# CZW123456/Quantized_Decoder_Polar_Codes

Measured on AMD Instinct MI355X. Metric: decoded frames/sec (N=1024, SCL-LUT L=8, Q=16) at 1/2/4/8 GPUs; BER match, higher is better.
Workload: dtype u8; 1 GPU; SCL-LUT N=1024 K=512 L=8 Q=16 (5G-NR PW code, no CRC); decoder=SCL-LUT, N=1024, K=512, L=8, v=16, luts=mindistortion, parallelism=dp1 (frames sharded by global frame id, RCCL counter all-reduce), engine=fast, lds_bytes_per_wave=7424, lds_from_depth=5, ops=266, prefix_ops=65, waves=5120

## Files before the change

### quantized_decoder_polar_codes_amd/csrc/qpd_capi_build.hpp

```cpp
#pragma once
#include <cstdlib>
#include <cstring>
#include <map>

#include "qpd_config.hpp"
#include "qpd_decoder.hpp"
#include "qpd_plan.hpp"
#include "qpd_schedule.hpp"

namespace qpd {
const void *fast_kernel_single(int kind, int sets);
const void *prefix_kernel(int kind, int sets, bool pw1);
const void *fast_kernel_scl(int sets, bool l8, bool w16);
const void *fast_kernel_scl_pw1(int sets, bool l8, bool w16);
const void *fast_kernel_fscl(int sets, bool l8, bool r1l);
const void *fast_kernel_fscl_pw1(int sets, bool l8, bool r1l);
const void *fast_kernel_fscl_w16(int sets, bool pw1);
const void *generic_kernel(int fam, int dom, bool wide);
const void *generic_list_kernel(int fam, int dom, bool wide);
const void *dmetric_kernel();
const void *fast_kernel_scl_st(int sets, bool l8, bool w16);
const void *fast_kernel_scl_pw1_st(int sets, bool l8, bool w16);
const void *fast_kernel_fscl_st(int sets, bool l8, bool r1l);
const void *fast_kernel_fscl_pw1_st(int sets, bool l8, bool r1l);
const void *fast_kernel_fscl_w16_st(int sets, bool pw1);
const void *fast_kernel_scl_ls(int sets, bool l8, bool w16);
const void *fast_kernel_scl_pw1_ls(int sets, bool l8, bool w16);
// ... 27 lines not shown
            default: return nullptr;
        }
    }
    switch (kind) {
        case QPD_SC_LUT:
        case QPD_FASTSC_LUT: return pw1 || r1l ? nullptr : qpd::fast_kernel_single(kind, sets);
        case QPD_SCL_LUT: return r1l ? nullptr : pw1 ? qpd::fast_kernel_scl_pw1(sets, l8, w16) : qpd::fast_kernel_scl(sets, l8, w16);
        case QPD_FASTSCL_LUT:
            if (w16) return r1l ? nullptr : qpd::fast_kernel_fscl_w16(sets, pw1);
            return pw1 ? qpd::fast_kernel_fscl_pw1(sets, l8, r1l) : qpd::fast_kernel_fscl(sets, l8, r1l);
        default: return nullptr;
    }
}
using qpd::generic_kernel;
using qpd::prefix_kernel;

int init_task_queue(qpd_decoder *d) {
    uint32_t v0 = 0;
    if (const char *e = getenv("QPD_TASK_BASE0")) v0 = (uint32_t)strtoull(e, nullptr, 0);
    const uint32_t init[2] = {v0, 0u};
    const int rc = upload(d->task_ctr, init, 2, d->hs);
    if (rc) return rc;
    d->task_base = v0;
    return QPD_OK;
}

#ifdef QPD_STAMPS
unsigned long long *stamp_buffer() {
    static std::mutex mu;
    static std::map<int, unsigned long long *> bufs;
// ... 138 lines not shown
    d->lds_bytes = H.lds_bytes;
    d->lds_tab_bytes = H.lds_tab_bytes;
    d->sets = H.sets;
    d->pfx_sets = H.pfx_sets;
    d->l8 = H.l8;
    d->w16 = H.w16;
    d->r1l = H.r1l;
    d->pw1 = H.pw1;
    d->pre = H.pre;
    d->pre_chunk = H.pre_chunk;
    for (int i = 0; i < 3; ++i) {
        d->pfx[i].nops = (int)H.pfx[i].size();
        d->pfx[i].rec = H.pfx_rec[i], d->pfx[i].pm = H.pfx_pm[i];
        d->pfx[i].paths = 1 << i;
    }
    F.nops = (int)H.ops.size();
    d->num_mops = F.nops + d->prefix_ops();
}

int upload_fast_plan(qpd_decoder *d, const qpd_plan::FastHostPlan &H) {
    int rc;
    if ((rc = upload(d->r1_rank, H.r1tab.data(), H.r1tab.size(), d->hs))) return rc;
    for (const auto &st : H.pfx)
        d->pfx_ops_host.insert(d->pfx_ops_host.end(), st.begin(), st.end());
    if (!d->pfx_ops_host.empty()) {
        if ((rc = upload(d->pfx_mops, d->pfx_ops_host.data(), d->pfx_ops_host.size(), d->hs))) return rc;
        d->main_ops_host = H.ops;
    }
    if ((rc = upload(d->mops, H.ops.data(), H.ops.size(), d->hs))) return rc;
    if ((rc = upload(d->f_tab, H.ft.data(), H.ft.size(), d->hs))) return rc;
    return upload(d->g_tab, H.gt.data(), H.gt.size(), d->hs);
}

int build_fast(qpd_decoder *d, const qpd_config *c, const Schedule &s) {
    qpd::FastPlan &F = d->fplan;
#ifdef QPD_STAMPS
    F.stamps = stamp_buffer();
#endif
    qpd_plan::FastHostPlan H;
    std::string err;
    int rc = qpd_plan::plan_fast(*c, d->n, d->L, s, qpd_plan::PlanSwitches::from_env(), H, err);
    if (rc) return fail(rc, err);
    adopt_fast_plan(d, c, s, H);
    if ((rc = upload_fast_plan(d, H))) return rc;
    const void *kfn = fast_kernel(d->kind, d->sets, d->l8, d->r1l, d->pw1, d->w16);
    if (!kfn) return fail(QPD_E_UNSUPPORTED, "fast plan: no decode kernel instantiation for this plan");
    if ((rc = check_no_static_lds(kfn, "fast decode kernel"))) return rc;
    if (d->kind == QPD_SCL_LUT || d->kind == QPD_FASTSCL_LUT) {
        const void *ksfn = fast_kernel(d->kind, d->sets, d->l8, d->r1l, d->pw1, d->w16, 1);
        if (!ksfn) return fail(QPD_E_UNSUPPORTED, "fast plan: no decode-status kernel instantiation for this plan");
        if ((rc = check_no_static_lds(ksfn, "fast decode-status kernel"))) return rc;
        if (d->L > 1 && d->L <= qpd_list::kMaxListOut) {
            const void *klfn = fast_kernel(d->kind, d->sets, d->l8, d->r1l, d->pw1, d->w16, 2);
            if (!klfn) return fail(QPD_E_UNSUPPORTED, "fast plan: no list-output kernel instantiation for this plan");
            if ((rc = check_no_static_lds(klfn, "fast list-output kernel"))) return rc;
        }
    }
    if (d->pfx[0].nops > 0 && d->pfx_sets == 2 &&
        (rc = check_no_static_lds(prefix_kernel(d->kind, d->pfx_sets, d->pw1), "fast prefix kernel")))
        return rc;
    const int64_t per_wave = (int64_t)d->sets * F.glb_rows * 64 * 4;
    int mw = c->max_waves;
    if (mw <= 0) {
        int per_cu = 0;
        const int ncu = device_cus();
        const hipError_t oe = hipOccupancyMaxActiveBlocksPerMultiprocessor(&per_cu, kfn, 64, d->lds_bytes);
        if (oe != hipSuccess || per_cu <= 0) per_cu = 16;
        mw = std::max(1, ncu) * per_cu;
    }
    mw = (int)std::max<int64_t>(1, std::min<int64_t>(mw, ((int64_t)2 << 30) / per_wave));
    d->max_waves = mw;
    d->scratch_bytes_per_wave = per_wave;
    QPD_HIP(hipMalloc(&d->fscratch.p, (size_t)per_wave * mw));
    F.r1_rank = (const uint16_t *)d->r1_rank.p;
    F.f_tab = (const uint32_t *)d->f_tab.p;
    F.g_tab = (const uint32_t *)d->g_tab.p;
// ... 88 lines not shown
```

### quantized_decoder_polar_codes_amd/csrc/qpd_capi_decode.hpp

```cpp
#pragma once
#include "qpd_capi_build.hpp"
#include "qpd_decoder.hpp"
#include "qpd_fast_pre.hpp"

namespace {

int import_stage(const qpd::MOp &m) { return m.node == 3 ? 1 : m.node == 2 ? 2 : 0; }

int patch_imports(qpd_decoder *d, hipStream_t st) {
    bool moved = false;
    for (const auto &sg : d->pfx) moved = moved || sg.patched != sg.buf.p;
    if (!moved) return QPD_OK;
    auto patch = [&](std::vector<qpd::MOp> &v) {
        for (qpd::MOp &m : v)
            if (m.type == qpd::OP_IMPORT && (m.flags & qpd::MF_XBUF)) {
                const uint64_t a = (uint64_t)(uintptr_t)d->pfx[import_stage(m)].buf.p;
                m.u_row = (int32_t)(uint32_t)a;
                m.r_row = (int32_t)(uint32_t)(a >> 32);
            }
    };
    patch(d->pfx_ops_host);
    patch(d->main_ops_host);
    QPD_HIP(hipMemcpyAsync(d->pfx_mops.p, d->pfx_ops_host.data(), d->pfx_ops_host.size() * sizeof(qpd::MOp),
                           hipMemcpyHostToDevice, st));
// ... 52 lines not shown
    qpd::DevPlan P = d->plan;
    P.task_base = d->task_base;
    status_at(d, out, P);
    list_at(d, out, P);
    const In *in_arg = in;
    void *args[] = {&P, &in_arg, &B, &out, &dmetric};
    const int rc = timed_launch(d, QPD_KC_DECODE, st, [&]() -> int {
        QPD_HIP(hipLaunchKernel(kfn, dim3(grid), dim3(64), args, 0, st));
        QPD_HIP(hipGetLastError());
        return QPD_OK;
    });
    if (!rc) d->task_base += (uint32_t)((B + d->plan.fpw - 1) / d->plan.fpw);
    return rc;
}

int fast_launch(qpd_decoder *d, qpd::FastPlan fp, const int32_t *in, int64_t Bc, uint8_t *out, hipStream_t st,
                bool prefix = false) {
    const int sets = prefix ? d->pfx_sets : d->sets;
    const int64_t tw = (int64_t)fp.fpw * sets;
    const bool status = !prefix && d->st_req.any(), list = !prefix && d->ls_req.any();
    const void *kfn = prefix ? prefix_kernel(d->kind, sets, d->pw1)
                             : fast_kernel(d->kind, d->sets, d->l8, d->r1l, d->pw1, d->w16, list ? 2 : status ? 1 : 0);
    if (!kfn) return fail(QPD_E_INVALID, "bad kind");
    qpd::FastStatus so{};
    if (status) status_at(d, out, so);
    if (list) list_at(d, out, so);
    const int64_t fgroups = (Bc + tw - 1) / tw;
    int fgrid = (int)std::min<int64_t>(fgroups, d->max_waves);
    if (!QPD_DYN) {
        const int64_t rounds = (fgroups + fgrid - 1) / fgrid;
        fgrid = (int)((fgroups + rounds - 1) / rounds);
    }
    const qpd::MOp *ops_arg = fp.ops;
    fp.task_base = d->task_base;
    void *args[] = {&fp, &in, &Bc, &out, &ops_arg, &so};
    const size_t lds = (size_t)((d->lds_bytes - d->lds_tab_bytes) / d->sets * sets + d->lds_tab_bytes);
    const int rc = timed_launch(d, prefix ? QPD_KC_PFX : QPD_KC_DECODE, st, [&]() -> int {
        QPD_HIP(hipLaunchKernel(kfn, dim3(fgrid), dim3(64), args, lds, st));
        QPD_HIP(hipGetLastError());
        return QPD_OK;
    });
    if (!rc) d->task_base += (uint32_t)fgroups;
    return rc;
}

constexpr int prefix_geo(int ps) { return (6 - ps) | (ps << 8); }
static_assert(prefix_geo(0) == 6 && prefix_geo(1) == (5 | (1 << 8)) && prefix_geo(2) == (4 | (2 << 8)), "stages 1, 1b, 2");

int decode_pre_rows(qpd_decoder *d, const uint32_t *rows, int64_t Bc, uint8_t *out, hipStream_t st) {
    qpd::FastPlan fp = d->fplan;
    fp.in_vec = 1;
    fp.in_shift = fp.n - 2;
    if (d->pfx[0].nops > 0) {
        int rc = QPD_OK;
        for (auto &sg : d->pfx)
            if (!rc && sg.nops > 0) rc = ensure_records(sg.buf, sg.cap, Bc, sg.rec, sg.paths);
        if (!rc) rc = patch_imports(d, st);
        if (rc) return rc;
        qpd::FastPlan pp = fp;
        const qpd::MOp *ops = (const qpd::MOp *)d->pfx_mops.p;
        for (const auto &sg : d->pfx) {
            if (sg.nops > 0) {
                const int ps = __builtin_ctz(sg.paths);
                pp.ops = ops;
                pp.nops = sg.nops;
                pp.gs = pp.L = sg.paths;
                pp.fpw = 64 >> ps;
                pp.pfx = (uint32_t *)sg.buf.p;
                pp.pfx_rec = sg.rec;
                pp.pfx_geo = prefix_geo(ps);
                pp.pm_off = sg.pm;
                if ((rc = fast_launch(d, pp, (const int32_t *)rows, Bc, nullptr, st, true))) return rc;
            }
            ops += sg.nops;
        }
    }
    return fast_launch(d, fp, (const int32_t *)rows, Bc, out, st);
}

int64_t reserve_pre_rows(qpd_decoder *d, int64_t B, int *rc) {
    return d->pre_rows.reserve(std::min<int64_t>(B, d->pre_chunk), (size_t)d->N, "pre-pass rows hipMalloc: ", rc);
}

int64_t reserve_symbols(qpd_decoder *d, DeviceChunk &buf, int64_t B, int64_t lim, const char *what, int *rc) {
    if (!lim) lim = std::max<int64_t>(1, ((int64_t)1 << 30) / ((int64_t)d->N * 4));
    return buf.reserve(std::min<int64_t>(B, lim), (size_t)d->N * sizeof(int32_t), what, rc);
}
// ... 123 lines not shown
```

### quantized_decoder_polar_codes_amd/csrc/qpd_decoder.hpp

```cpp
#pragma once
#include <hip/hip_runtime.h>

#include <algorithm>
#include <cstdint>
#include <memory>
#include <mutex>
#include <string>
#include <utility>
#include <vector>

#include "qpd.h"
#include "qpd_generic.hip"
#include "qpd_fast_plan.hpp"
#include "qpd_chunk.hpp"
#include "qpd_host.hpp"
#include "qpd_status.hpp"
#include "qpd_list.hpp"

namespace {

thread_local std::string g_err;

int fail(int code, const std::string &msg) {
    g_err = msg;
// ... 78 lines not shown
    DevPlan plan{};
    qpd::FastPlan fplan{};
    DeviceBuf f_tab, g_tab, fscratch, mops, r1_rank, task_ctr;
    int num_mops = 0;
    DeviceBuf pfx_mops;
    int pfx_sets = 1;
    struct PrefixStage {
        int nops = 0;
        int rec = 0, pm = 0;
        int paths = 1;
        DeviceBuf buf;
        size_t cap = 0;
        const void *patched = nullptr;
    } pfx[3];
    int prefix_ops() const { return pfx[0].nops + pfx[1].nops + pfx[2].nops; }
    std::vector<qpd::MOp> pfx_ops_host, main_ops_host;
    std::vector<Op> ops_host;
    DeviceBuf lut_f, f_base, lut_g, g_base, vcl, ops, info_pos, scratch, err;
    DeviceBuf r_f, r_g, q_bnd, q_rec, bnd_off, bnd_len, rec_off, rec_len;
    DeviceBuf h_in, h_out, h_st;
    size_t h_in_bytes = 0, h_out_bytes = 0, h_st_bytes = 0;
    hipStream_t hs = nullptr;
    void *pin = nullptr;
    size_t pin_bytes = 0;
    std::mutex mu;
    hipEvent_t last_ev = nullptr;
    hipStream_t last_st = nullptr;
    bool last_valid = false;
    uint32_t task_base = 0;
    std::unique_ptr<qpd_host::Plan> hplan;
// ... 100 lines not shown
```

### quantized_decoder_polar_codes_amd/csrc/qpd_fast.hip

```cpp
#pragma once
#include "qpd_fast_switches.hpp"

#include "qpd_fast_plan.hpp"
#include "qpd_fast_lookup.hpp"
#include "qpd_fast_select.hpp"
#include "qpd_fast_bot.hpp"
#include "qpd_fast_special.hpp"

#define QPD_TAIL_PLAIN 0
#define QPD_TAIL_ST 1
#define QPD_TAIL_LIST 2

#if defined(QPD_LIST_UNIT)
#define QPD_ST QPD_TAIL_LIST
#define QPD_UNIT_FN(f) f##_ls
#elif defined(QPD_STATUS_UNIT)
#define QPD_ST QPD_TAIL_ST
#define QPD_UNIT_FN(f) f##_st
#else
#define QPD_ST QPD_TAIL_PLAIN
#define QPD_UNIT_FN(f) f
#endif

namespace qpd {

template <int KIND, int NS, bool L8, bool R1L = false, bool PFX = false, bool PW1 = false, bool W16 = false,
          int ST = QPD_TAIL_PLAIN>
__global__ __launch_bounds__(64, NS == 3 ? QPD_WPE3
                                : W16 ? QPD_WPE_W16
                                : NS == 2 ? (KIND == K_SCL_LUT && !PFX ? QPD_WPE2_SCL : KIND == K_FASTSCL_LUT ? QPD_WPE2_FSCL : QPD_WPE2)
                                : KIND == K_FASTSCL_LUT ? QPD_WPE_FSCL : QPD_WPE1) void lut_fast_kernel(FastPlan P, const int32_t *__restrict__ in, int64_t B,
                                                               uint8_t *__restrict__ out,
                                                               const MOp *__restrict__ ops, FastStatus SO) {
    constexpr bool kList = (KIND == K_SCL_LUT || KIND == K_FASTSCL_LUT);
    static_assert(!W16 || (!L8 && (KIND == K_SCL_LUT || (KIND == K_FASTSCL_LUT && !R1L && !PFX))),
                  "W16: SCL-LUT / FastSCL-LUT list sizes 9..16");
    static_assert(!ST || (kList && !PFX), "ST: the list kinds' decode kernels");
    constexpr int LM = L8 ? 8 : W16 ? 16 : 0;
    constexpr bool kLazy = QPD_BOT3_LAZY && kList;
    constexpr bool kFast = (KIND == K_FASTSC_LUT || KIND == K_FASTSCL_LUT) && !(QPD_EXP_FSCL & 256);
    constexpr bool kChan = !(PW1 && KIND == K_SCL_LUT);
    extern __shared__ __attribute__((aligned(16))) uint32_t lds_dyn[];
    constexpr bool kLdsTab = kList && NS >= 2 && !QPD_EXP_NO_LDSTAB;
    constexpr int kTabWords = kLdsTab ? 192 : 0;
    uint8_t *const tb = (uint8_t *)lds_dyn;
    uint32_t *const lds_rows = lds_dyn + kTabWords;
    const int sstride = 64;
    int *const sel_all = (int *)(lds_rows + NS * P.lds_rows * 64);
    Mem Mv[NS];
    {
        uint32_t *const slab = P.scratch + (size_t)blockIdx.x * NS * P.glb_rows * 64;
        const __amdgpu_buffer_rsrc_t rs =
            __builtin_amdgcn_make_buffer_rsrc(slab, 0, NS * P.glb_rows * 256 * QPD_EXP_SLABMUL, 0x00020000);
#pragma unroll
        for (int s = 0; s < NS; ++s) {
            Mv[s].lds = lds_rows + s * 64;
            Mv[s].gp = slab + s * 64;
            Mv[s].rs = rs;
            Mv[s].so = s * 256;
            Mv[s].ns = NS;
        }
    }
    const int gs = P.gs;
    const int L = kList ? P.L : 1;
    const int N = P.N;
    const int64_t fpw = P.fpw;
    const int64_t ntasks = (B + NS * fpw - 1) / (NS * fpw);
    const double kInf = __builtin_huge_val();

    for (int64_t task = blockIdx.x; task < ntasks;
         task = QPD_DYN ? (int64_t)gridDim.x + wave_take(P.task_ctr, P.task_base) : task + gridDim.x) {
#ifdef QPD_POISON
        for (int i = threadIdx.x; i < NS * (P.lds_rows * 64 + kSelInts); i += 64) lds_rows[i] = (uint32_t)QPD_POISON;
        for (int r = 0; r < NS * P.glb_rows; ++r) Mv[0].gp[r * 64 + threadIdx.x] = (uint32_t)QPD_POISON;
        wave_sync();
#endif
        PathT<PW1> stv[NS];
        {
            const int lane = threadIdx.x, gl = lane & (gs - 1);
            uint64_t self = 0;
            for (int d = 0; d < kMaxDepth; ++d) self |= (uint64_t)gl << (4 * d);
#pragma unroll
            for (int s = 0; s < NS; ++s) {
                stv[s].pm = (gl == 0) ? 0.0 : kInf;
                stv[s].ps = self;
                stv[s].U() = self;
            }
        }
#ifdef QPD_STAMPS
        uint64_t stamp_acc = 0, stamp_cnt = 0;
#endif
        MOp nxt = ops[0];
        Pre pre = fetch_pre(P, nxt, threadIdx.x, threadIdx.x < P.v ? threadIdx.x : 0);
        for (int oi = 0; oi < P.nops; ++oi) {
            int lane = threadIdx.x;
            asm volatile("" : "+v"(lane));
            const int gl = lane & (gs - 1);
            const int gbase = lane & ~(gs - 1);
            const int vlane = lane < P.v ? lane : 0;
            const int32_t *yv[NS];
            const int gsh = __builtin_ctz(gs);
            if (nxt.flags & (MF_CHAN | MF_PRE)) {
#pragma unroll
                for (int s = 0; s < NS; ++s) {
                    int64_t f = (task * NS + s) * fpw + (lane >> gsh);
                    if (f >= B) f = B - 1;
                    yv[s] = in + (f << P.in_shift);
                }
            } else {
#pragma unroll
                for (int s = 0; s < NS; ++s) yv[s] = in;
            }
            if (nxt.flags & MF_SYNC) wave_sync();
            const MOp op = nxt;
            const Pre cur = pre;
#ifdef QPD_STAMPS
            __builtin_amdgcn_s_waitcnt(0);
            const uint64_t stamp_t0 = __builtin_amdgcn_s_memtime();
#endif
            if (oi + 1 < P.nops) {
                nxt = ops[oi + 1];
                if (!kLazy || op.type != OP_BOT3) pre = fetch_pre(P, nxt, lane, vlane);
            }
            const int fl = op.flags;
            auto run_special = [&]() {
              if constexpr (kFast) {
                  if constexpr (KIND == K_FASTSCL_LUT && L8) {
                    if ((op.type == OP_R0 || op.type == OP_REP) && !(QPD_EXP_FSCL & 512)) {
                        r0rep_multi<kLdsTab, R1L>(P, Mv, op, stv, sel_all, sstride, gl, gbase, lane, cur.T2, tb);
                        return;
                    }
                    if (op.type == OP_R1 && (op.cnt <= stl::kThreshold || (fl & MF_R1_LDS)) && !(QPD_EXP_FSCL & 1024)) {
                        r1_multi<kLdsTab, R1L>(P, Mv, op, stv, sel_all, sstride, gl, gbase, lane, lds_rows, cur.T2, tb);
                        return;
                    }
                    if constexpr (!R1L) return;
// ... 5 lines not shown
                                               L, lane, lds_rows);
                    rotate_sets(stv);
                  }
#else
#pragma unroll
                  for (int s = 0; s < NS; ++s)
                    special_op<kList, LM, R1L>(P, Mv[s], op, stv[s], sel_all + sstride * s, NS * sstride, gl, gbase, L, lane,
                                               lds_rows);
#endif
              }
            };
            switch (op.type) {
                case OP_BOT3:
                    if constexpr (KIND == K_FASTSCL_LUT && L8 && !QPD_EXP_NO_BOTX) {
                        if (fl & MF_BOTX) {
                            if (kLazy && oi + 1 < P.nops) pre = fetch_pre(P, nxt, lane, vlane);
                            botx_op<kLdsTab, kChan>(P, Mv, op, yv, stv, cur.T, cur.T2, gl, gbase, L, sel_all, sstride, lane, tb);
                            break;
                        }
                    }
                    bot3_op<kList, LM, kLazy, kLdsTab, kChan>(P, Mv, op, yv, stv, cur.T, cur.T2, gl, gbase, L, sel_all, sstride, lane, [&]() {
                        if (oi + 1 < P.nops) pre = fetch_pre(P, nxt, lane, vlane);
                    }, tb);
                    break;
                case OP_F:
                case OP_G: {
                    int src[NS], usrc[NS];
#pragma unroll
                    for (int s = 0; s < NS; ++s) {
                        src[s] = gbase + pfield(stv[s].ps, op.sh_src);
                        usrc[s] = gbase + pfield(stv[s].U(), op.sh_u);
                    }
                    if constexpr (kLdsTab) {
                        if (fl & MF_FF) {
                            const int key = ((fl & MF_DST_LDS) ? 1 : 0) | ((fl & MF_FF_DL) ? 2 : 0);
                            stage_tab(tb, cur.T, op.type == OP_F ? (lane & 31) : gtab_dw(lane));
                            stage_tab(tb + 512, cur.T2, lane & 31);
// ... 112 lines not shown
#pragma unroll
                        for (int s = 0; s < NS; ++s) stv[s].U() = pset(stv[s].U(), op.sh_dst, gl);
                    }
                    break;
                }
                case OP_IMPORT:
                    if constexpr (KIND == K_SCL_LUT) {
                        const int live = op.tab2;
#pragma unroll
                        for (int s = 0; s < NS; ++s) {
                            const bool dl = fl & MF_DST_LDS;
                            if (fl & MF_ZERO) {
                                for (int w = 0; w < op.cnt; ++w) Mv[s].st(dl, op.dst_row + w, lane, 0u);
                                continue;
                            }
                            int64_t f = (task * NS + s) * fpw + (lane >> gsh);
                            if (f >= B) f = B - 1;
                            const int G = op.vrow & 255;
                            const uint32_t *src = (const uint32_t *)(((uint64_t)(uint32_t)op.r_row << 32) | (uint32_t)op.u_row) +
                                                  (((f >> G) * op.tab) << 6) + ((f & ((1 << G) - 1)) << (op.vrow >> 8)) +
                                                  (gl < live ? gl : 0);
                            if (fl & MF_PM) {
                                const uint64_t b = (uint64_t)src[op.src_row << 6] | ((uint64_t)src[(op.src_row + 1) << 6] << 32);
                                stv[s].pm = gl < live ? __builtin_bit_cast(double, b) : kInf;
                                            } else {
                                for (int w = 0; w < op.cnt; ++w) Mv[s].st(dl, op.dst_row + w, lane, src[(op.src_row + w) << 6]);
                            }
                        }
                    }
                    break;
                case OP_EXPORT:
                    if constexpr (KIND == K_SCL_LUT && PFX) {
#pragma unroll
                        for (int s = 0; s < NS; ++s) {
                            const int64_t f = (task * NS + s) * fpw + (lane >> gsh);
                            const int at = (fl & MF_VIA_PS)   ? gbase + pfield(stv[s].ps, op.sh_src)
                                           : (fl & MF_VIA_PU) ? gbase + pfield(stv[s].U(), op.sh_src)
                                                              : lane;
                            const int G = P.pfx_geo & 255;
                            uint32_t *dst = P.pfx + (((f >> G) * P.pfx_rec) << 6) + ((f & ((1 << G) - 1)) << (P.pfx_geo >> 8)) + gl;
                            for (int w = 0; w < op.cnt; ++w) {
                                const uint32_t x = Mv[s].ld(fl & MF_SRC_LDS, op.src_row + w, at);
                                if (f < B) dst[(op.dst_row + w) << 6] = x;
                            }
                        }
                    }
                    break;
                default:
                    if constexpr (kFast) run_special();
                    break;
// ... 7 lines not shown
                const int cls = op.type == OP_F ? dd : op.type == OP_G ? 8 + dd : op.type == OP_COMB ? 16 + dd
                              : op.type == OP_BOT3 ? ((fl & MF_BOTX) ? 30 : 24) : (op.type == OP_LEAF_L || op.type == OP_LEAF_R) ? 25
                              : 26 + (op.type - OP_R0) % 4;
#else
                const int cls = op.type == OP_R1 ? 24 + (op.cnt > 16) + (op.cnt > 8) : 2 * op.type + ((fl & MF_SYNC) ? 1 : 0);
#endif
                if ((int)(threadIdx.x & 31) == cls) stamp_acc += dt;
                if ((int)(threadIdx.x & 31) == cls) stamp_cnt += 1;
            }
#endif
        }
        if constexpr (PFX) {
            const int gl = threadIdx.x & (gs - 1);
#pragma unroll
            for (int s = 0; s < NS; ++s) {
                const int64_t f = (task * NS + s) * fpw + (threadIdx.x >> __builtin_ctz(gs));
                const int G = P.pfx_geo & 255;
                uint32_t *dst = P.pfx + (((f >> G) * P.pfx_rec) << 6) + ((f & ((1 << G) - 1)) << (P.pfx_geo >> 8)) + gl;
                const uint64_t b = __builtin_bit_cast(uint64_t, stv[s].pm);
                if (f < B) {
                    dst[P.pm_off << 6] = (uint32_t)b;
                    dst[(P.pm_off + 1) << 6] = (uint32_t)(b >> 32);
                }
            }
            wave_sync();
            continue;
        }
#ifdef QPD_STAMPS
        __builtin_amdgcn_s_waitcnt(0);
        const uint64_t stamp_t2 = __builtin_amdgcn_s_memtime();
#endif
// ... 159 lines not shown
        wave_sync();
#ifdef QPD_STAMPS
        __builtin_amdgcn_s_waitcnt(0);
        if (threadIdx.x == 31) stamp_acc += __builtin_amdgcn_s_memtime() - stamp_t2;
        if (threadIdx.x == 31) stamp_cnt += 1;
        if (threadIdx.x < 32) {
            atomicAdd(&P.stamps[threadIdx.x], (unsigned long long)stamp_acc);
            atomicAdd(&P.stamps[32 + threadIdx.x], (unsigned long long)stamp_cnt);
        }
#endif
    }
}

#define lut_prefix_kernel(KIND, NS, PW1) lut_fast_kernel<KIND, NS, false, false, true, PW1>

}
```

### quantized_decoder_polar_codes_amd/csrc/qpd_fast_plan.hpp

```cpp
#pragma once
#include "qpd_fast_switches.hpp"

#include <hip/hip_runtime.h>
#include <stdint.h>

#include "qpd_mop.hpp"

namespace qpd {

struct FastPlan {
    int32_t N, n, K, L, v, gs, fpw, nops, max_r1;
    int32_t in_vec;
    int32_t in_shift;
    int32_t out_k;
    int32_t ca_A, crc_n;
    uint32_t crc_q;
    const uint32_t *info_mask;
    int32_t lds_rows, glb_rows, lds_from;
    int32_t R0_row, R0_lds;
    int32_t H_row, K_row, I_row;
    const uint32_t *f_tab;
    const uint32_t *g_tab;
    const double *vcl;
    const MOp *ops;
    const int32_t *info_pos;
    const uint16_t *r1_rank;
    uint32_t *scratch;
    int32_t *err;
    uint32_t *task_ctr;
    uint32_t task_base;
    uint32_t *pfx;
    int32_t pfx_rec, pfx_geo, pm_off;
#ifdef QPD_STAMPS
    unsigned long long *stamps;
#endif
};

struct FastStatus {
    uint32_t crc_mask;
    double *st_metric;
    uint8_t *st_pass;
    uint8_t *ls_bits;
    double *ls_metric;
    uint8_t *ls_pass;
    int32_t *ls_chosen;
};

struct Mem {
    uint32_t *lds;
    uint32_t *gp;
    __amdgpu_buffer_rsrc_t rs;
// ... 39 lines not shown
```

### quantized_decoder_polar_codes_amd/csrc/qpd_fast_switches.hpp

```cpp
#pragma once


#ifndef QPD_WPE1
#define QPD_WPE1 6
#endif
#ifndef QPD_WPE_FSCL
#define QPD_WPE_FSCL 6
#endif
#ifndef QPD_WPE2
#define QPD_WPE2 4
#endif
#ifndef QPD_WPE2_SCL
#define QPD_WPE2_SCL 5
#endif
#ifndef QPD_WPE2_FSCL
#define QPD_WPE2_FSCL 4
#endif
#ifndef QPD_WPE3
#define QPD_WPE3 3
#endif
#ifndef QPD_WPE_W16
#define QPD_WPE_W16 4
#endif

#ifndef QPD_LUT_PACK2
#define QPD_LUT_PACK2 1
#endif
#ifndef QPD_LUT_OPAQUE
#define QPD_LUT_OPAQUE 1
#endif
#ifndef QPD_LUT_OPAQUE_XY
#define QPD_LUT_OPAQUE_XY 1
#endif

#ifndef QPD_BOT3_LAZY
#define QPD_BOT3_LAZY 1
#endif
// ... 48 lines not shown
```

### quantized_decoder_polar_codes_amd/csrc/qpd_k_fast.hip

```cpp
#include "qpd_fast.hip"
#include "qpd.h"

namespace qpd {

const void *fast_kernel_single(int kind, int sets) {
#define QPD_FK(K, S) reinterpret_cast<const void *>(&lut_fast_kernel<K, S, false>)
    switch (kind) {
        case QPD_SC_LUT: return sets == 2 ? QPD_FK(K_SC_LUT, 2) : QPD_FK(K_SC_LUT, 1);
        case QPD_FASTSC_LUT: return sets == 2 ? QPD_FK(K_FASTSC_LUT, 2) : QPD_FK(K_FASTSC_LUT, 1);
        default: return nullptr;
    }
#undef QPD_FK
}

const void *prefix_kernel(int kind, int sets, bool pw1) {
    if (kind != QPD_SCL_LUT) return nullptr;
    if (pw1)
        return sets == 2 ? reinterpret_cast<const void *>(&lut_prefix_kernel(K_SCL_LUT, 2, true))
                         : reinterpret_cast<const void *>(&lut_prefix_kernel(K_SCL_LUT, 1, true));
    return sets == 2 ? reinterpret_cast<const void *>(&lut_prefix_kernel(K_SCL_LUT, 2, false))
                     : reinterpret_cast<const void *>(&lut_prefix_kernel(K_SCL_LUT, 1, false));
}

}
```

### quantized_decoder_polar_codes_amd/csrc/qpd_mop.hpp

```cpp
#pragma once
#include <stdint.h>

#include "qpd_types.hpp"

namespace qpd {

constexpr int OP_BOT3 = 9;
constexpr int OP_IMPORT = 10;
constexpr int OP_EXPORT = 11;

enum MopFlag : int32_t {
    MF_SRC_LDS = 1,
    MF_DST_LDS = 2,
    MF_U_LDS = 4,
    MF_TO_R = 8,
    MF_SYNC = 16,
    MF_R_LDS = 32,
    MF_CHAN = 64,
    MF_R1_LDS = 128,
    MF_PRE = 256,
    MF_GSEL = 512,
    MF_BFG = 1024,
    MF_BG = 2048,
    MF_BCOMB = 4096,
// ... 2 lines not shown
    MF_PM = 32768,
    MF_VIA_PS = 65536,
    MF_VIA_PU = 131072,
    MF_XBUF = 262144,
    MF_FF = 524288,
    MF_FF_DL = 1048576,
    MF_BC2 = 2097152,
    MF_BC2_ULDS = 4194304,
    MF_BC2_DLDS = 8388608,
    MF_BC2_TOR = 16777216,
    MF_BOTX = 33554432,
    MF_R1_RK = 67108864,
    MF_SFG = 134217728,
    MF_SGG = 268435456,
    MF_SCOMB = 536870912,
};

struct MOp {
    int32_t type, flags, d, node;
    int32_t cnt;
    int32_t src_row;
    int32_t dst_row;
    int32_t u_row;
    int32_t r_row;
    int32_t sh_src;
    int32_t sh_u;
    int32_t sh_dst;
    int32_t tab;
    int32_t vrow;
    int32_t tab2;
// ... 11 lines not shown
```

### quantized_decoder_polar_codes_amd/csrc/qpd_plan.hpp

```cpp
#pragma once
#include <algorithm>
#include <climits>
#include <cmath>
#include <cstdint>
#include <cstdlib>
#include <cstring>
#include <string>
#include <vector>

#include "qpd.h"
#include "qpd_mop.hpp"
#include "qpd_schedule.hpp"
#include "stl_sort.hpp"

namespace qpd_plan {

using qpd_sched::Schedule;
using qpd_sched::special_of;

struct PlanSwitches {
    static constexpr int kUnset = INT_MIN;
    int sets = 0;
    int lds_budget = kUnset;
    int64_t pre_chunk = 0;
    int pfx_sets = 0;
    bool pfx1b = false;
    bool no_pre = false;
    bool no_bfuse = false;
    bool no_botx = false;
    bool no_trim = false;
    bool no_pfx = false;
    bool no_pfx2 = false;
    bool no_ff = false;
    bool no_bc2 = false;
    bool no_pw1 = false;
    bool no_vuni = false;
    bool no_r1rk = false;
    bool no_sfold = false;
#ifdef QPD_DIAG
    int botx_sel = -1;
#endif
    static PlanSwitches from_env() {
        PlanSwitches w;
        auto on = [](const char *name) { return getenv(name) != nullptr; };
        if (const char *e = getenv("QPD_SETS")) {
            w.sets = std::min(2, std::max(1, atoi(e)));
#ifdef QPD_SETS3
            if (atoi(e) == 3) w.sets = 3;
#endif
        }
        if (const char *e = getenv("QPD_LDS_BUDGET")) w.lds_budget = atoi(e);
        if (const char *e = getenv("QPD_PRE_CHUNK")) w.pre_chunk = std::max<int64_t>(1, atoll(e));
        if (const char *e = getenv("QPD_PFX_SETS")) w.pfx_sets = std::max(1, atoi(e));
        w.pfx1b = on("QPD_PFX1B");
        w.no_pre = on("QPD_NO_PRE");
        w.no_bfuse = on("QPD_NO_BFUSE");
        w.no_botx = on("QPD_NO_BOTX");
        w.no_trim = on("QPD_NO_TRIM");
        w.no_pfx = on("QPD_NO_PFX");
        w.no_pfx2 = on("QPD_NO_PFX2");
        w.no_ff = on("QPD_NO_FF");
        w.no_bc2 = on("QPD_NO_BC2");
        w.no_pw1 = on("QPD_NO_PW1");
        w.no_vuni = on("QPD_NO_VUNI");
        w.no_r1rk = on("QPD_NO_R1RK");
        w.no_sfold = on("QPD_NO_SFOLD");
#ifdef QPD_DIAG
        if (const char *e = getenv("QPD_BOTX_SEL")) w.botx_sel = atoi(e);
#endif
        return w;
    }
};

struct FastLayout {
    int D = 0;
    int S[qpd::kMaxDepth + 1] = {}, U[qpd::kMaxDepth + 1] = {}, R[qpd::kMaxDepth + 1] = {};
    int lds_base[qpd::kMaxDepth + 2] = {};
    int lds_end = 0;
    bool pre = false;
    bool bfuse = false;
    int ns = 1;
    bool botx = false;
    bool lds(int dd) const { return dd >= D; }
};

struct FastHostPlan {
    std::vector<qpd::MOp> ops;
    std::vector<qpd::MOp> pfx[3];
    int pfx_rec[3] = {}, pfx_pm[3] = {};
    std::vector<uint16_t> r1tab;
    std::vector<uint32_t> ft, gt;
    int lds_from = 0, lds_rows = 0, glb_rows = 0;
    int R0_row = 0, R0_lds = 0;
    int H_row = 0, K_row = 0, I_row = 0;
    int lds_bytes = 0, lds_tab_bytes = 0;
    int lds_budget = 0;
    int sets = 1, pfx_sets = 1;
    bool l8 = false;
    bool w16 = false;
    bool r1l = false;
    bool pw1 = false;
    bool pre = false;
    int64_t pre_chunk = 0;
    FastLayout layout;
    bool use[3][qpd::kMaxDepth + 1];
};

inline bool bot3_plain(int kind, const int32_t *node_type, int n, int d, int node) {
    if (n < 3 || d != n - 3) return false;
    for (int dd = d; dd < n; ++dd)
// ... 546 lines not shown
    if (sb > s1 && sb < s2 && sw.pfx1b && live_in(ops, sb, own, liveb)) {
        std::vector<MOp> impb, expb;
        path_records(liveb, 5, 1, 3, impb, expb, P.pfx_rec[1], P.pfx_pm[1]);
        P.pfx[1] = imp1;
        P.pfx[1].insert(P.pfx[1].end(), ops.begin() + s1, ops.begin() + sb);
        P.pfx[1].insert(P.pfx[1].end(), expb.begin(), expb.end());
        imp1 = impb;
        s1 = sb;
    }
    P.pfx[2] = imp1;
    P.pfx[2].insert(P.pfx[2].end(), ops.begin() + s1, ops.begin() + s2);
    P.pfx[2].insert(P.pfx[2].end(), exp2.begin(), exp2.end());
    rest = imp2;
    rest.insert(rest.end(), ops.begin() + s2, ops.end());
    return true;
}

#ifndef QPD_DEFAULT_SETS
#define QPD_DEFAULT_SETS 2
#endif
constexpr int kDefaultSets = QPD_DEFAULT_SETS;

template <class Fn>
void pointer_fields(qpd::MOp &m, int &bc_u, int &bc_dst, Fn &&fn) {
    using namespace qpd;
    bc_u = m.pad1 & 255;
    bc_dst = (m.pad1 >> 8) & 255;
    const int fl = m.flags;
    const bool src_row = !(fl & (MF_CHAN | MF_PRE));
    switch (m.type) {
// ... 229 lines not shown
    P.r1l = false;
    for (const qpd::MOp &m : mops)
        if (c.kind == QPD_FASTSCL_LUT &&
            ((m.type == qpd::OP_R1 &&
              ((m.cnt > qpd::stl::kThreshold && !(m.flags & qpd::MF_R1_LDS)) || (P.l8 && !(m.flags & qpd::MF_R1_RK)))) ||
             (P.l8 && (m.type == qpd::OP_R0 || m.type == qpd::OP_REP) && !(m.flags & qpd::MF_VUNI))))
            P.r1l = true;
    if (c.kind == QPD_FASTSCL_LUT && P.w16 && P.r1l) {
        err = "fast engine, FastSCL-LUT with L > 8: an R1 node of more than 32 elements, or of more than 16 "
              "without room for its argsort in LDS, is not served (use the generic engine)";
        return QPD_E_UNSUPPORTED;
    }
    const bool pw1_ok = c.kind == QPD_SCL_LUT ? NS <= 2 && Ly.pre
                                              : (c.kind == QPD_FASTSCL_LUT && ((NS == 2 && P.l8 && !P.r1l) || P.w16));
    P.pw1 = pw1_ok && !sw.no_pw1 && compact_pointer_fields(lists);
    for (const qpd::MOp &m : mops)
        if ((m.type == qpd::OP_F || m.type == qpd::OP_G) && (m.flags & qpd::MF_SRC_LDS) && !(m.flags & qpd::MF_DST_LDS)) {
            err = "fast plan: an f/g op reads LDS rows and writes slab rows";
            return QPD_E_INVALID;
        }
    pack_tables(c, P.ft, P.gt);
    return QPD_OK;
}

}
```

Before: 58.04 million frames/s.

## Merge frozen-prefix stage kernels into one launch with on-chip handoff

Fuses the path-1 and path-4 prefix stages of the SCL-LUT decoder into a single kernel. Each task first runs the stage-0 ops, then loops over the phases that expand the list, handing the records over through LDS (or a scratch slab) instead of a global record buffer. This removes one kernel launch plus the global export/import round trip for stage-0 records. In exchange the prefix kernel needs more LDS or scratch per wave, which can lower occupancy, and the task loop gains phase-dependent control flow.

```diff
diff --git a/quantized_decoder_polar_codes_amd/csrc/qpd_capi_build.hpp b/quantized_decoder_polar_codes_amd/csrc/qpd_capi_build.hpp
--- a/quantized_decoder_polar_codes_amd/csrc/qpd_capi_build.hpp
+++ b/quantized_decoder_polar_codes_amd/csrc/qpd_capi_build.hpp
@@ -11,6 +11,7 @@
 namespace qpd {
 const void *fast_kernel_single(int kind, int sets);
 const void *prefix_kernel(int kind, int sets, bool pw1);
+const void *prefix_merged_kernel(int kind, int sets, bool pw1);
 const void *fast_kernel_scl(int sets, bool l8, bool w16);
 const void *fast_kernel_scl_pw1(int sets, bool l8, bool w16);
 const void *fast_kernel_fscl(int sets, bool l8, bool r1l);
@@ -68,6 +69,7 @@
 }
 using qpd::generic_kernel;
 using qpd::prefix_kernel;
+using qpd::prefix_merged_kernel;
 
 int init_task_queue(qpd_decoder *d) {
     uint32_t v0 = 0;
@@ -236,6 +238,11 @@
         d->pfx[i].rec = H.pfx_rec[i], d->pfx[i].pm = H.pfx_pm[i];
         d->pfx[i].paths = 1 << i;
     }
+    d->pfx_merged = H.merged;
+    d->mrg_nops = (int)H.mrg.size();
+    d->mrg_n1 = H.mrg_n1;
+    d->mrg_lds_bytes = H.mrg_lds_bytes;
+    d->mrg_glb_rows = H.mrg_glb_rows;
     F.nops = (int)H.ops.size();
     d->num_mops = F.nops + d->prefix_ops();
 }
@@ -249,6 +256,7 @@
         if ((rc = upload(d->pfx_mops, d->pfx_ops_host.data(), d->pfx_ops_host.size(), d->hs))) return rc;
         d->main_ops_host = H.ops;
     }
+    if (H.merged && (rc = upload(d->mrg_mops, H.mrg.data(), H.mrg.size(), d->hs))) return rc;
     if ((rc = upload(d->mops, H.ops.data(), H.ops.size(), d->hs))) return rc;
     if ((rc = upload(d->f_tab, H.ft.data(), H.ft.size(), d->hs))) return rc;
     return upload(d->g_tab, H.gt.data(), H.gt.size(), d->hs);
@@ -278,10 +286,13 @@
             if ((rc = check_no_static_lds(klfn, "fast list-output kernel"))) return rc;
         }
     }
-    if (d->pfx[0].nops > 0 && d->pfx_sets == 2 &&
-        (rc = check_no_static_lds(prefix_kernel(d->kind, d->pfx_sets, d->pw1), "fast prefix kernel")))
-        return rc;
-    const int64_t per_wave = (int64_t)d->sets * F.glb_rows * 64 * 4;
+    if (d->pfx[0].nops > 0) {
+        if ((rc = check_no_static_lds(prefix_kernel(d->kind, d->pfx_sets, d->pw1), "fast prefix kernel"))) return rc;
+        if (d->pfx_merged &&
+            (rc = check_no_static_lds(prefix_merged_kernel(d->kind, d->pfx_sets, d->pw1), "fast merged prefix kernel")))
+            return rc;
+    }
+    const int64_t per_wave = std::max((int64_t)d->sets * F.glb_rows, d->pfx_merged ? (int64_t)d->pfx_sets * d->mrg_glb_rows : 0) * 64 * 4;
     int mw = c->max_waves;
     if (mw <= 0) {
         int per_cu = 0;
diff --git a/quantized_decoder_polar_codes_amd/csrc/qpd_capi_decode.hpp b/quantized_decoder_polar_codes_amd/csrc/qpd_capi_decode.hpp
--- a/quantized_decoder_polar_codes_amd/csrc/qpd_capi_decode.hpp
+++ b/quantized_decoder_polar_codes_amd/csrc/qpd_capi_decode.hpp
@@ -90,13 +90,17 @@
     return rc;
 }
 
+enum FastLaunch { FL_DECODE, FL_PREFIX, FL_PREFIX_MERGED };
+
 int fast_launch(qpd_decoder *d, qpd::FastPlan fp, const int32_t *in, int64_t Bc, uint8_t *out, hipStream_t st,
-                bool prefix = false) {
+                FastLaunch what = FL_DECODE) {
+    const bool prefix = what != FL_DECODE;
     const int sets = prefix ? d->pfx_sets : d->sets;
     const int64_t tw = (int64_t)fp.fpw * sets;
     const bool status = !prefix && d->st_req.any(), list = !prefix && d->ls_req.any();
-    const void *kfn = prefix ? prefix_kernel(d->kind, sets, d->pw1)
-                             : fast_kernel(d->kind, d->sets, d->l8, d->r1l, d->pw1, d->w16, list ? 2 : status ? 1 : 0);
+    const void *kfn = what == FL_PREFIX_MERGED ? prefix_merged_kernel(d->kind, sets, d->pw1)
+                      : prefix               ? prefix_kernel(d->kind, sets, d->pw1)
+                                             : fast_kernel(d->kind, d->sets, d->l8, d->r1l, d->pw1, d->w16, list ? 2 : status ? 1 : 0);
     if (!kfn) return fail(QPD_E_INVALID, "bad kind");
     qpd::FastStatus so{};
     if (status) status_at(d, out, so);
@@ -110,7 +114,8 @@
     const qpd::MOp *ops_arg = fp.ops;
     fp.task_base = d->task_base;
     void *args[] = {&fp, &in, &Bc, &out, &ops_arg, &so};
-    const size_t lds = (size_t)((d->lds_bytes - d->lds_tab_bytes) / d->sets * sets + d->lds_tab_bytes);
+    const size_t lds = what == FL_PREFIX_MERGED ? (size_t)d->mrg_lds_bytes
+                                                : (size_t)((d->lds_bytes - d->lds_tab_bytes) / d->sets * sets + d->lds_tab_bytes);
     const int rc = timed_launch(d, prefix ? QPD_KC_PFX : QPD_KC_DECODE, st, [&]() -> int {
         QPD_HIP(hipLaunchKernel(kfn, dim3(fgrid), dim3(64), args, lds, st));
         QPD_HIP(hipGetLastError());
@@ -130,13 +135,29 @@
     if (d->pfx[0].nops > 0) {
         int rc = QPD_OK;
         for (auto &sg : d->pfx)
-            if (!rc && sg.nops > 0) rc = ensure_records(sg.buf, sg.cap, Bc, sg.rec, sg.paths);
+            if (!rc && sg.nops > 0 && !(d->pfx_merged && &sg == &d->pfx[0]))
+                rc = ensure_records(sg.buf, sg.cap, Bc, sg.rec, sg.paths);
         if (!rc) rc = patch_imports(d, st);
         if (rc) return rc;
         qpd::FastPlan pp = fp;
         const qpd::MOp *ops = (const qpd::MOp *)d->pfx_mops.p;
+        if (d->pfx_merged) {
+            const auto &sg = d->pfx[2];
+            const int ps = __builtin_ctz(sg.paths);
+            pp.ops = (const qpd::MOp *)d->mrg_mops.p;
+            pp.nops = d->mrg_nops;
+            pp.pfx_n1 = d->mrg_n1;
+            pp.gs = pp.L = sg.paths;
+            pp.fpw = 64;
+            pp.glb_rows = d->mrg_glb_rows;
+            pp.pfx = (uint32_t *)sg.buf.p;
+            pp.pfx_rec = sg.rec;
+            pp.pfx_geo = prefix_geo(ps);
+            pp.pm_off = sg.pm;
+            if ((rc = fast_launch(d, pp, (const int32_t *)rows, Bc, nullptr, st, FL_PREFIX_MERGED))) return rc;
+        }
         for (const auto &sg : d->pfx) {
-            if (sg.nops > 0) {
+            if (sg.nops > 0 && !d->pfx_merged) {
                 const int ps = __builtin_ctz(sg.paths);
                 pp.ops = ops;
                 pp.nops = sg.nops;
@@ -146,7 +167,7 @@
                 pp.pfx_rec = sg.rec;
                 pp.pfx_geo = prefix_geo(ps);
                 pp.pm_off = sg.pm;
-                if ((rc = fast_launch(d, pp, (const int32_t *)rows, Bc, nullptr, st, true))) return rc;
+                if ((rc = fast_launch(d, pp, (const int32_t *)rows, Bc, nullptr, st, FL_PREFIX))) return rc;
             }
             ops += sg.nops;
         }
diff --git a/quantized_decoder_polar_codes_amd/csrc/qpd_decoder.hpp b/quantized_decoder_polar_codes_amd/csrc/qpd_decoder.hpp
--- a/quantized_decoder_polar_codes_amd/csrc/qpd_decoder.hpp
+++ b/quantized_decoder_polar_codes_amd/csrc/qpd_decoder.hpp
@@ -116,6 +116,9 @@
         const void *patched = nullptr;
     } pfx[3];
     int prefix_ops() const { return pfx[0].nops + pfx[1].nops + pfx[2].nops; }
+    bool pfx_merged = false;
+    DeviceBuf mrg_mops;
+    int mrg_nops = 0, mrg_n1 = 0, mrg_lds_bytes = 0, mrg_glb_rows = 0;
     std::vector<qpd::MOp> pfx_ops_host, main_ops_host;
     std::vector<Op> ops_host;
     DeviceBuf lut_f, f_base, lut_g, g_base, vcl, ops, info_pos, scratch, err;
diff --git a/quantized_decoder_polar_codes_amd/csrc/qpd_fast.hip b/quantized_decoder_polar_codes_amd/csrc/qpd_fast.hip
--- a/quantized_decoder_polar_codes_amd/csrc/qpd_fast.hip
+++ b/quantized_decoder_polar_codes_amd/csrc/qpd_fast.hip
@@ -25,7 +25,7 @@
 namespace qpd {
 
 template <int KIND, int NS, bool L8, bool R1L = false, bool PFX = false, bool PW1 = false, bool W16 = false,
-          int ST = QPD_TAIL_PLAIN>
+          int ST = QPD_TAIL_PLAIN, bool MRG = false>
 __global__ __launch_bounds__(64, NS == 3 ? QPD_WPE3
                                 : W16 ? QPD_WPE_W16
                                 : NS == 2 ? (KIND == K_SCL_LUT && !PFX ? QPD_WPE2_SCL : KIND == K_FASTSCL_LUT ? QPD_WPE2_FSCL : QPD_WPE2)
@@ -36,6 +36,7 @@
     static_assert(!W16 || (!L8 && (KIND == K_SCL_LUT || (KIND == K_FASTSCL_LUT && !R1L && !PFX))),
                   "W16: SCL-LUT / FastSCL-LUT list sizes 9..16");
     static_assert(!ST || (kList && !PFX), "ST: the list kinds' decode kernels");
+    static_assert(!MRG || (PFX && KIND == K_SCL_LUT), "MRG: the merged frozen-prefix kernel");
     constexpr int LM = L8 ? 8 : W16 ? 16 : 0;
     constexpr bool kLazy = QPD_BOT3_LAZY && kList;
     constexpr bool kFast = (KIND == K_FASTSC_LUT || KIND == K_FASTSCL_LUT) && !(QPD_EXP_FSCL & 256);
@@ -61,15 +62,27 @@
             Mv[s].ns = NS;
         }
     }
-    const int gs = P.gs;
-    const int L = kList ? P.L : 1;
+    int gs = P.gs;
+    int L = kList ? P.L : 1;
     const int N = P.N;
     const int64_t fpw = P.fpw;
     const int64_t ntasks = (B + NS * fpw - 1) / (NS * fpw);
     const double kInf = __builtin_huge_val();
 
+    int ph = 0;
     for (int64_t task = blockIdx.x; task < ntasks;
-         task = QPD_DYN ? (int64_t)gridDim.x + wave_take(P.task_ctr, P.task_base) : task + gridDim.x) {
+         task = (MRG && (ph = ph < P.gs ? ph + 1 : 0) != 0) ? task
+                : QPD_DYN ? (int64_t)gridDim.x + wave_take(P.task_ctr, P.task_base)
+                          : task + gridDim.x) {
+        const MOp *opl = ops;
+        int nops = P.nops;
+        int foff = 0;
+        if constexpr (MRG) {
+            gs = L = ph ? P.gs : 1;
+            opl = ph ? ops + P.pfx_n1 : ops;
+            nops = ph ? P.nops - P.pfx_n1 : P.pfx_n1;
+            foff = ph ? (ph - 1) * (64 / P.gs) : 0;
+        }
 #ifdef QPD_POISON
         for (int i = threadIdx.x; i < NS * (P.lds_rows * 64 + kSelInts); i += 64) lds_rows[i] = (uint32_t)QPD_POISON;
         for (int r = 0; r < NS * P.glb_rows; ++r) Mv[0].gp[r * 64 + threadIdx.x] = (uint32_t)QPD_POISON;
@@ -90,9 +103,9 @@
 #ifdef QPD_STAMPS
         uint64_t stamp_acc = 0, stamp_cnt = 0;
 #endif
-        MOp nxt = ops[0];
+        MOp nxt = opl[0];
         Pre pre = fetch_pre(P, nxt, threadIdx.x, threadIdx.x < P.v ? threadIdx.x : 0);
-        for (int oi = 0; oi < P.nops; ++oi) {
+        for (int oi = 0; oi < nops; ++oi) {
             int lane = threadIdx.x;
             asm volatile("" : "+v"(lane));
             const int gl = lane & (gs - 1);
@@ -103,7 +116,7 @@
             if (nxt.flags & (MF_CHAN | MF_PRE)) {
 #pragma unroll
                 for (int s = 0; s < NS; ++s) {
-                    int64_t f = (task * NS + s) * fpw + (lane >> gsh);
+                    int64_t f = (task * NS + s) * fpw + (lane >> gsh) + foff;
                     if (f >= B) f = B - 1;
                     yv[s] = in + (f << P.in_shift);
                 }
@@ -118,8 +131,8 @@
             __builtin_amdgcn_s_waitcnt(0);
             const uint64_t stamp_t0 = __builtin_amdgcn_s_memtime();
 #endif
-            if (oi + 1 < P.nops) {
-                nxt = ops[oi + 1];
+            if (oi + 1 < nops) {
+                nxt = opl[oi + 1];
                 if (!kLazy || op.type != OP_BOT3) pre = fetch_pre(P, nxt, lane, vlane);
             }
             const int fl = op.flags;
@@ -155,13 +168,13 @@
                 case OP_BOT3:
                     if constexpr (KIND == K_FASTSCL_LUT && L8 && !QPD_EXP_NO_BOTX) {
                         if (fl & MF_BOTX) {
-                            if (kLazy && oi + 1 < P.nops) pre = fetch_pre(P, nxt, lane, vlane);
+                            if (kLazy && oi + 1 < nops) pre = fetch_pre(P, nxt, lane, vlane);
                             botx_op<kLdsTab, kChan>(P, Mv, op, yv, stv, cur.T, cur.T2, gl, gbase, L, sel_all, sstride, lane, tb);
                             break;
                         }
                     }
                     bot3_op<kList, LM, kLazy, kLdsTab, kChan>(P, Mv, op, yv, stv, cur.T, cur.T2, gl, gbase, L, sel_all, sstride, lane, [&]() {
-                        if (oi + 1 < P.nops) pre = fetch_pre(P, nxt, lane, vlane);
+                        if (oi + 1 < nops) pre = fetch_pre(P, nxt, lane, vlane);
                     }, tb);
                     break;
                 case OP_F:
@@ -304,6 +317,19 @@
                                 for (int w = 0; w < op.cnt; ++w) Mv[s].st(dl, op.dst_row + w, lane, 0u);
                                 continue;
                             }
+                            if constexpr (MRG) {
+                                const bool sl = fl & MF_SRC_LDS;
+                                const int col = foff + (lane >> gsh);
+                                if (fl & MF_PM) {
+                                    const uint64_t b = (uint64_t)Mv[s].ldv(sl, op.src_row, col) |
+                                                       ((uint64_t)Mv[s].ldv(sl, op.src_row + 1, col) << 32);
+                                    stv[s].pm = gl < live ? __builtin_bit_cast(double, b) : kInf;
+                                } else {
+                                    for (int w = 0; w < op.cnt; ++w)
+                                        Mv[s].st(dl, op.dst_row + w, lane, Mv[s].ldv(sl, op.src_row + w, col));
+                                }
+                                continue;
+                            }
                             int64_t f = (task * NS + s) * fpw + (lane >> gsh);
                             if (f >= B) f = B - 1;
                             const int G = op.vrow & 255;
@@ -323,7 +349,21 @@
                     if constexpr (KIND == K_SCL_LUT && PFX) {
 #pragma unroll
                         for (int s = 0; s < NS; ++s) {
-                            const int64_t f = (task * NS + s) * fpw + (lane >> gsh);
+                            if constexpr (MRG) {
+                                if (fl & MF_HAND) {
+                                    const bool hl = fl & MF_DST_LDS;
+                                    if (fl & MF_PM) {
+                                        const uint64_t b = __builtin_bit_cast(uint64_t, stv[s].pm);
+                                        Mv[s].st(hl, op.dst_row, lane, (uint32_t)b);
+                                        Mv[s].st(hl, op.dst_row + 1, lane, (uint32_t)(b >> 32));
+                                    } else {
+                                        for (int w = 0; w < op.cnt; ++w)
+                                            Mv[s].st(hl, op.dst_row + w, lane, Mv[s].ld(fl & MF_SRC_LDS, op.src_row + w, lane));
+                                    }
+                                    continue;
+                                }
+                            }
+                            const int64_t f = (task * NS + s) * fpw + (lane >> gsh) + foff;
                             const int at = (fl & MF_VIA_PS)   ? gbase + pfield(stv[s].ps, op.sh_src)
                                            : (fl & MF_VIA_PU) ? gbase + pfield(stv[s].U(), op.sh_src)
                                                               : lane;
@@ -361,7 +401,8 @@
             const int gl = threadIdx.x & (gs - 1);
 #pragma unroll
             for (int s = 0; s < NS; ++s) {
-                const int64_t f = (task * NS + s) * fpw + (threadIdx.x >> __builtin_ctz(gs));
+                if (MRG && ph == 0) break;
+                const int64_t f = (task * NS + s) * fpw + (threadIdx.x >> __builtin_ctz(gs)) + foff;
                 const int G = P.pfx_geo & 255;
                 uint32_t *dst = P.pfx + (((f >> G) * P.pfx_rec) << 6) + ((f & ((1 << G) - 1)) << (P.pfx_geo >> 8)) + gl;
                 const uint64_t b = __builtin_bit_cast(uint64_t, stv[s].pm);
@@ -551,4 +592,7 @@
 
 #define lut_prefix_kernel(KIND, NS, PW1) lut_fast_kernel<KIND, NS, false, false, true, PW1>
 
+#define lut_prefix_merged_kernel(KIND, NS, PW1) \
+    lut_fast_kernel<KIND, NS, false, false, true, PW1, false, QPD_TAIL_PLAIN, true>
+
 }
diff --git a/quantized_decoder_polar_codes_amd/csrc/qpd_fast_plan.hpp b/quantized_decoder_polar_codes_amd/csrc/qpd_fast_plan.hpp
--- a/quantized_decoder_polar_codes_amd/csrc/qpd_fast_plan.hpp
+++ b/quantized_decoder_polar_codes_amd/csrc/qpd_fast_plan.hpp
@@ -31,10 +31,15 @@
     uint32_t task_base;
     uint32_t *pfx;
     int32_t pfx_rec, pfx_geo, pm_off;
+    int32_t pfx_n1;
 #ifdef QPD_STAMPS
     unsigned long long *stamps;
 #endif
 };
+
+#ifndef QPD_STAMPS
+static_assert(sizeof(FastPlan) == 208, "FastPlan: pfx_n1 fills the tail padding");
+#endif
 
 struct FastStatus {
     uint32_t crc_mask;
diff --git a/quantized_decoder_polar_codes_amd/csrc/qpd_fast_switches.hpp b/quantized_decoder_polar_codes_amd/csrc/qpd_fast_switches.hpp
--- a/quantized_decoder_polar_codes_amd/csrc/qpd_fast_switches.hpp
+++ b/quantized_decoder_polar_codes_amd/csrc/qpd_fast_switches.hpp
@@ -21,6 +21,10 @@
 #endif
 #ifndef QPD_WPE_W16
 #define QPD_WPE_W16 4
+#endif
+
+#ifndef QPD_PFX_MERGE
+#define QPD_PFX_MERGE 1
 #endif
 
 #ifndef QPD_LUT_PACK2
diff --git a/quantized_decoder_polar_codes_amd/csrc/qpd_k_fast.hip b/quantized_decoder_polar_codes_amd/csrc/qpd_k_fast.hip
--- a/quantized_decoder_polar_codes_amd/csrc/qpd_k_fast.hip
+++ b/quantized_decoder_polar_codes_amd/csrc/qpd_k_fast.hip
@@ -22,4 +22,13 @@
                      : reinterpret_cast<const void *>(&lut_prefix_kernel(K_SCL_LUT, 1, false));
 }
 
+const void *prefix_merged_kernel(int kind, int sets, bool pw1) {
+    if (kind != QPD_SCL_LUT) return nullptr;
+    if (pw1)
+        return sets == 2 ? reinterpret_cast<const void *>(&lut_prefix_merged_kernel(K_SCL_LUT, 2, true))
+                         : reinterpret_cast<const void *>(&lut_prefix_merged_kernel(K_SCL_LUT, 1, true));
+    return sets == 2 ? reinterpret_cast<const void *>(&lut_prefix_merged_kernel(K_SCL_LUT, 2, false))
+                     : reinterpret_cast<const void *>(&lut_prefix_merged_kernel(K_SCL_LUT, 1, false));
 }
+
+}
diff --git a/quantized_decoder_polar_codes_amd/csrc/qpd_mop.hpp b/quantized_decoder_polar_codes_amd/csrc/qpd_mop.hpp
--- a/quantized_decoder_polar_codes_amd/csrc/qpd_mop.hpp
+++ b/quantized_decoder_polar_codes_amd/csrc/qpd_mop.hpp
@@ -40,6 +40,7 @@
     MF_SFG = 134217728,
     MF_SGG = 268435456,
     MF_SCOMB = 536870912,
+    MF_HAND = 1073741824,
 };
 
 struct MOp {
diff --git a/quantized_decoder_polar_codes_amd/csrc/qpd_plan.hpp b/quantized_decoder_polar_codes_amd/csrc/qpd_plan.hpp
--- a/quantized_decoder_polar_codes_amd/csrc/qpd_plan.hpp
+++ b/quantized_decoder_polar_codes_amd/csrc/qpd_plan.hpp
@@ -9,6 +9,7 @@
 #include <vector>
 
 #include "qpd.h"
+#include "qpd_fast_switches.hpp"
 #include "qpd_mop.hpp"
 #include "qpd_schedule.hpp"
 #include "stl_sort.hpp"
@@ -37,6 +38,7 @@
     bool no_vuni = false;
     bool no_r1rk = false;
     bool no_sfold = false;
+    int8_t pfx_merge = 0;
 #ifdef QPD_DIAG
     int botx_sel = -1;
 #endif
@@ -65,6 +67,7 @@
         w.no_vuni = on("QPD_NO_VUNI");
         w.no_r1rk = on("QPD_NO_R1RK");
         w.no_sfold = on("QPD_NO_SFOLD");
+        if (const char *e = getenv("QPD_PFX_MERGE")) w.pfx_merge = atoi(e) ? 1 : -1;
 #ifdef QPD_DIAG
         if (const char *e = getenv("QPD_BOTX_SEL")) w.botx_sel = atoi(e);
 #endif
@@ -94,6 +97,12 @@
     int R0_row = 0, R0_lds = 0;
     int H_row = 0, K_row = 0, I_row = 0;
     int lds_bytes = 0, lds_tab_bytes = 0;
+    std::vector<qpd::MOp> mrg;
+    int mrg_n1 = 0;
+    int hand_row = 0, hand_rows = 0;
+    bool hand_lds = false;
+    int mrg_lds_bytes = 0, mrg_glb_rows = 0;
+    bool merged = false;
     int lds_budget = 0;
     int sets = 1, pfx_sets = 1;
     bool l8 = false;
@@ -670,6 +679,56 @@
     rest = imp2;
     rest.insert(rest.end(), ops.begin() + s2, ops.end());
     return true;
+}
+
+inline int prefix_wave_lds(int pfx_sets) { return 160 * 1024 / (4 * (pfx_sets >= 2 ? QPD_WPE2 : QPD_WPE1)); }
+
+inline int prefix_lds_bytes(const FastHostPlan &P) {
+    return (P.lds_bytes - P.lds_tab_bytes) / P.sets * P.pfx_sets + P.lds_tab_bytes;
+}
+
+inline void plan_prefix_merged(FastHostPlan &P) {
+    using namespace qpd;
+    P.mrg.clear();
+    P.mrg_n1 = P.hand_row = P.hand_rows = P.mrg_lds_bytes = P.mrg_glb_rows = 0;
+    P.hand_lds = false;
+    if (P.pfx[0].empty() || P.pfx[2].empty() || !P.pfx[1].empty()) return;
+    for (const MOp &m : P.pfx[2])
+        if (m.type == OP_IMPORT && (m.flags & MF_XBUF) && m.node != 1) return;
+    P.hand_rows = P.pfx_rec[0];
+    const int hand_bytes = P.pfx_sets * P.hand_rows * 256;
+    P.hand_lds = prefix_lds_bytes(P) + hand_bytes <= prefix_wave_lds(P.pfx_sets);
+    P.hand_row = P.hand_lds ? P.lds_rows + kSelInts / 64 : P.glb_rows;
+    P.mrg_lds_bytes = prefix_lds_bytes(P) + (P.hand_lds ? hand_bytes : 0);
+    P.mrg_glb_rows = P.glb_rows + (P.hand_lds ? 0 : P.hand_rows);
+    for (MOp m : P.pfx[0]) {
+        if (m.type == OP_EXPORT) {
+            m.flags |= MF_HAND | (P.hand_lds ? MF_DST_LDS : 0);
+            m.dst_row += P.hand_row;
+        }
+        P.mrg.push_back(m);
+    }
+    MOp pm = blank_op(OP_EXPORT);
+    pm.flags = MF_HAND | MF_PM | (P.hand_lds ? MF_DST_LDS : 0);
+    pm.dst_row = P.hand_row + P.pfx_pm[0];
+    P.mrg.push_back(pm);
+    P.mrg_n1 = (int)P.mrg.size();
+    for (MOp m : P.pfx[2]) {
+        if (m.type == OP_IMPORT && (m.flags & MF_XBUF)) {
+            m.flags |= MF_HAND | (P.hand_lds ? MF_SRC_LDS : 0);
+            m.src_row += P.hand_row;
+        }
+        P.mrg.push_back(m);
+    }
+}
+
+template <class Fn>
+void hand_rows_of(const qpd::MOp &m, Fn &&fn) {
+    using namespace qpd;
+    if (!(m.flags & MF_HAND)) return;
+    const int cnt = (m.flags & MF_PM) ? 2 : m.cnt;
+    if (m.type == OP_EXPORT) fn(true, (m.flags & MF_DST_LDS) != 0, m.dst_row, cnt);
+    if (m.type == OP_IMPORT) fn(false, (m.flags & MF_SRC_LDS) != 0, m.src_row, cnt);
 }
 
 #ifndef QPD_DEFAULT_SETS
@@ -929,6 +988,8 @@
     const bool pw1_ok = c.kind == QPD_SCL_LUT ? NS <= 2 && Ly.pre
                                               : (c.kind == QPD_FASTSCL_LUT && ((NS == 2 && P.l8 && !P.r1l) || P.w16));
     P.pw1 = pw1_ok && !sw.no_pw1 && compact_pointer_fields(lists);
+    plan_prefix_merged(P);
+    P.merged = !P.mrg.empty() && (sw.pfx_merge ? sw.pfx_merge > 0 : QPD_PFX_MERGE != 0);
     for (const qpd::MOp &m : mops)
         if ((m.type == qpd::OP_F || m.type == qpd::OP_G) && (m.flags & qpd::MF_SRC_LDS) && !(m.flags & qpd::MF_DST_LDS)) {
             err = "fast plan: an f/g op reads LDS rows and writes slab rows";
```

After: 58.40 million frames/s (median of 6 runs). No clear change (+0.6%).
